# valeoai/PAFUSE

Measured on AMD Instinct MI355X. Metric: hypotheses/sec through DDIM loop (H3WB 133-kp, P=20, T=10), higher is better.
Workload: dtype bf16x3 (every fp32 GEMM operand as the exact sum of three bf16 slices, six bf16 MFMA products per fp32-equivalent product, fp32 accumulate; activations, LayerNorm, softmax, attention and everything in memory fp32; the residual stream stored centred on its row means)

## Files before the change

### pafuse_amd/csrc/kernels.hpp

```cpp
#pragma once
#include <hip/hip_runtime.h>
#include <stdint.h>

#include <utility>

namespace pafuse {

typedef float f32x16 __attribute__((ext_vector_type(16)));
typedef float f32x4 __attribute__((ext_vector_type(4)));

constexpr int BK = 32;
constexpr int LDK = 36;

typedef __bf16 bf16x8 __attribute__((ext_vector_type(8)));
__device__ __forceinline__ bf16x8 to_bf16x8(const f32x4 lo, const f32x4 hi) {
    bf16x8 v;
#pragma unroll
    for (int i = 0; i < 4; ++i) v[i] = (__bf16)lo[i], v[4 + i] = (__bf16)hi[i];
    return v;
}

#ifdef PAFUSE_MFMA_K8
typedef __bf16 bf16x4_t __attribute__((ext_vector_type(4)));
typedef short s16x4_t __attribute__((ext_vector_type(4)));
// ... 1238 lines not shown
            }
            static_for<NG>([&](auto G) {
                constexpr int g = decltype(G)::value;
                constexpr int nt = g % NT;
                constexpr bool SPL = g < NT && ABL < 3 && NS2 == 2;
                constexpr int q0 = SPL ? (4 * nt) / NT : 0, q1 = SPL ? (4 * (nt + 1)) / NT : 0;
                if constexpr (g + 1 < NG) {
                    load_w(std::integral_constant<int, g + 1>{});
                    if constexpr (g == 0 && NS2 == 2) {
                        asm volatile("s_waitcnt lgkmcnt(3)"
                                     : "+v"(wf[0][0]), "+v"(wf[0][1]), "+v"(wf[0][2]), "+v"(b_lo), "+v"(b_hi));
    #pragma unroll
                        for (int q = 0; q < 4; ++q) {
                            sp[q].x0 = __builtin_bit_cast(float, q < 2 ? b_lo[2 * q] : b_hi[2 * q - 4]);
                            sp[q].x1 = __builtin_bit_cast(float, q < 2 ? b_lo[2 * q + 1] : b_hi[2 * q - 3]);
                        }
                    } else {
                        asm volatile("s_waitcnt lgkmcnt(3)" : "+v"(wf[g & 1][0]), "+v"(wf[g & 1][1]), "+v"(wf[g & 1][2]));
                    }
                } else {
                    asm volatile("s_waitcnt lgkmcnt(0)" : "+v"(wf[g & 1][0]), "+v"(wf[g & 1][1]), "+v"(wf[g & 1][2]));
                }
                const u32x4(&w)[3] = wf[g & 1];
                auto mm = [&](int wi, int ai) {
                    PAFUSE_PIN_ACC(acc[nt]);
                    acc[nt] = mfma_bf16_k16(__builtin_bit_cast(bf16x8, w[wi]), __builtin_bit_cast(bf16x8, cur[ai]), acc[nt]);
                };
                auto pins = [&]() {
    #pragma unroll
                    for (int q = q0; q < q1; ++q) PAFUSE_PIN_PAIR(sp[q]);
                };
                pins();
                mm(0, 2);
                {
                    constexpr int PER = (CNT + NG - 1) / NG, j0 = g * PER, j1 = (g + 1) * PER < CNT ? (g + 1) * PER : CNT;
                    if constexpr (j0 < j1 && ABL < 2) {
                        asm volatile("" ::: "memory");
                        if (refill) {
    #pragma unroll
                            for (int j = j0; j < j1; ++j) issue_piece(kn, stn, j);
                        }
                        asm volatile("" ::: "memory");
                    }
                }
    #pragma unroll
                for (int q = q0; q < q1; ++q) sp[q].template stage<0>();
                pins();
                mm(2, 0);
    #pragma unroll
                for (int q = q0; q < q1; ++q) sp[q].template stage<1>();
                pins();
                mm(1, 1);
    #pragma unroll
                for (int q = q0; q < q1; ++q) sp[q].template stage<2>();
                pins();
                mm(0, 1);
    #pragma unroll
                for (int q = q0; q < q1; ++q) sp[q].template stage<3>();
                pins();
                mm(1, 0);
    #pragma unroll
                for (int q = q0; q < q1; ++q) {
                    sp[q].template stage<4>();
                    nxt[0][q] = sp[q].s0, nxt[1][q] = sp[q].s1, nxt[2][q] = sp[q].s2;
                }
                pins();
                mm(0, 0);
                if constexpr (g == NT - 1 && ABL < 3 && NS2 == 2) cur[0] = nxt[0], cur[1] = nxt[1], cur[2] = nxt[2];
                if constexpr (g == NT - 1 && ABL >= 3 && NS2 == 2) {
    #pragma unroll
                    for (int q = 0; q < 4; ++q)
                        cur[0][q] = cur[2][q] = __builtin_bit_cast(uint32_t, sp[q].x0), cur[1][q] = __builtin_bit_cast(uint32_t, sp[q].x1);
                }
            });
    #undef PAFUSE_PIN_ACC
    #undef PAFUSE_PIN_PAIR
            __builtin_amdgcn_s_setprio(0);
        }
    }
    PAFUSE_STAMP(1);
    __syncthreads();
    constexpr int VEC = EPI == EPI_BIAS ? 0 : (7 * BM * WN + 3) / 4 * 4;
    if constexpr (VEC > 0) {
        static_assert((size_t)(VEC + 5 * BN) * sizeof(float) <= (size_t)NSTAGE * T::STAGE_BYTES, "epilogue vectors must fit the ring");
        const float* const src[5] = {p.bias, p.post_w, p.post_b, p.next_w, p.next_b};
#pragma unroll
        for (int v = 0; v < 5; ++v)
            if (src[v])
                for (int i = tid; i < BN / 4; i += T::NTHR)
                    *reinterpret_cast<f32x4*>(smem + VEC + v * BN + 4 * i) = *reinterpret_cast<const f32x4*>(src[v] + n0 + 4 * i);
        __syncthreads();
    }
    if constexpr (ABL == 4) {
        float sacc = 0.f;
#pragma unroll
        for (int nt = 0; nt < NT; ++nt)
#pragma unroll
            for (int i = 0; i < 16; ++i) sacc += acc[nt][i];
        if (sacc == 123.456f) p.out[0] = sacc;
        return;
    }
    if constexpr (EPI == EPI_ROWLN && SLAB) {
        constexpr size_t RINGF = (size_t)NSTAGE * T::STAGE_BYTES / sizeof(float);
        constexpr auto need = [](int nth) { return (size_t)VEC + 5 * BN + (size_t)NW * 32 * (32 * nth + 4); };
        constexpr int NTH = (NT % 2 == 0 && need(2) <= RINGF) ? 2 : 1;
        static_assert(need(NTH) <= RINGF, "epilogue scratch must fit the ring");
        epilogue_rows_h<WN, NT, BM, NW, NTH, false, 2>(acc, p, m0, n0, wm, wn, r, h, wave, lane, smem, 1.0f);
    } else {
        epilogue_row_per_lane<WN, NT, BM, EPI, VEC>(acc, p, m0, n0, wm, wn, r, h, smem);
    }
}

template <int WM, int WN, int NT, int EPI, int NSTAGE, int MINW, int ABL = 0, int BKC = 32>
__global__ void __launch_bounds__(WM* WN * 64, MINW) gemm_dma_kernel(const GemmParams p) {
    PAFUSE_XQ_GUARD();
    extern __shared__ __attribute__((aligned(16))) float smem[];
    gemm_dma_tile<WM, WN, NT, EPI, NSTAGE, ABL, BKC>(p, blockIdx.x, gridDim.x, smem);
}

constexpr int GROUP_MAX = 4;
struct GroupedGemmParams {
    GemmParams p[GROUP_MAX];
    int first[GROUP_MAX + 1];
    int n;
};

template <int EPI>
__global__ void __launch_bounds__(256, 2) grouped_rowln_kernel(const GroupedGemmParams g) {
    PAFUSE_XQ_GUARD();
    extern __shared__ __attribute__((aligned(16))) float smem[];
    const int b = blockIdx.x;
    int s = 0;
#pragma unroll
    for (int i = 1; i < GROUP_MAX; ++i)
        if (i < g.n && b >= g.first[i]) s = i;
    const GemmParams& p = g.p[s];
    const int lb = b - g.first[s], nb = g.first[s + 1] - g.first[s];
    switch (p.N) {
        case 384: gemm_dma_tile<2, 2, 6, EPI, 2, 0, 16, false>(p, lb, nb, smem); break;
        case 256: gemm_dma_tile<2, 2, 4, EPI, 2, 0, 16, false>(p, lb, nb, smem); break;
        case 224: gemm_dma_tile<4, 1, 7, EPI, 2, 0, 16, false>(p, lb, nb, smem); break;
        default: break;
    }
}

struct AttnParams {
    const float* qkv;
    float* o;
    uint8_t* o_h;
    int64_t nseq;
    int L, C, heads, d;
    int64_t group, group_stride, seq_stride, tok_stride;
    float scale;
};

template <int ITEMS>
__device__ __forceinline__ void attn_item(int64_t i, int64_t nseq, int heads, int64_t& seq, int& head) {
    if (nseq % 8 == 0 && ((nseq / 8) * heads) % ITEMS == 0) {
        const int64_t blk = i / ITEMS;
        const int lo = (int)(blk % 8);
        const int64_t u = (blk / 8) * ITEMS + (i % ITEMS);
        head = (int)(u % heads);
        seq = (u / heads) * 8 + lo;
    } else {
        seq = i / heads;
        head = (int)(i % heads);
    }
}

template <int LP, int DP, int NW>
__global__ void __launch_bounds__(NW * 64) attn_kernel(const AttnParams p) {
    PAFUSE_XQ_GUARD();
    constexpr int QT = LP / 16, KT = LP / 16, CT = DP / 16, SD = DP / 16, ITEMS = NW / QT, LDV = DP + 4;
    constexpr int NTHR = NW * 64, C4 = DP / 4;
    static_assert(NW % QT == 0, "waves must be a multiple of the query tiles");
    extern __shared__ __attribute__((aligned(16))) float smem[];
    float* Ks = smem;
    float* Vs = smem + ITEMS * LP * LDV;
    const int tid = threadIdx.x, lane = tid & 63, wave = tid >> 6;
    const int64_t nitems = p.nseq * p.heads;
    const int C3 = 3 * p.C;

    const int il = wave / QT, qt = wave % QT;
    const int64_t item = (int64_t)blockIdx.x * ITEMS + il;
    const bool mine = item < nitems;
    int64_t seq = 0;
    int head = 0;
    if (mine) attn_item<ITEMS>(item, p.nseq, p.heads, seq, head);
    const int64_t base = (seq / p.group) * p.group_stride + (seq % p.group) * p.seq_stride;
    const int l15 = lane & 15, g = lane >> 4;
    f32x4 qf[SD];
    {
        const int q = qt * 16 + l15;
#pragma unroll
        for (int s = 0; s < SD; ++s) {
            qf[s] = f32x4{0.f, 0.f, 0.f, 0.f};
            if (mine && q < p.L && 16 * s + 4 * g < p.d)
                qf[s] = *reinterpret_cast<const f32x4*>(p.qkv + (base + q * p.tok_stride) * C3 + head * p.d + 16 * s +
                                                        4 * g);
        }
    }
    for (int sl = 0; sl < ITEMS; ++sl) {
        const int64_t it2 = (int64_t)blockIdx.x * ITEMS + sl;
        const bool ok = it2 < nitems;
        int64_t seq2 = 0;
        int head2 = 0;
        if (ok) attn_item<ITEMS>(it2, p.nseq, p.heads, seq2, head2);
        const int64_t base2 = (seq2 / p.group) * p.group_stride + (seq2 % p.group) * p.seq_stride;
        for (int idx = tid; idx < LP * C4; idx += NTHR) {
            const int t = idx / C4, c4 = idx % C4;
            f32x4 kv = {0.f, 0.f, 0.f, 0.f}, vv = {0.f, 0.f, 0.f, 0.f};
            if (ok && t < p.L && c4 * 4 < p.d) {
                const float* src = p.qkv + (base2 + t * p.tok_stride) * C3 + head2 * p.d + c4 * 4;
                kv = *reinterpret_cast<const f32x4*>(src + p.C);
                vv = *reinterpret_cast<const f32x4*>(src + 2 * p.C);
            }
            *reinterpret_cast<f32x4*>(Ks + (sl * LP + t) * LDV + c4 * 4) = kv;
            *reinterpret_cast<f32x4*>(Vs + (sl * LP + t) * LDV + c4 * 4) = vv;
        }
    }
    __syncthreads();
    if (!mine) return;
    const float* Kb = Ks + il * LP * LDV;
    const float* Vb = Vs + il * LP * LDV;
    f32x4 sc[KT];
#pragma unroll
    for (int kt = 0; kt < KT; ++kt) sc[kt] = f32x4{0.f, 0.f, 0.f, 0.f};
#pragma unroll
    for (int s = 0; s < SD; ++s) {
        f32x4 kf[KT];
#pragma unroll
        for (int kt = 0; kt < KT; ++kt)
            kf[kt] = *reinterpret_cast<const f32x4*>(Kb + (kt * 16 + l15) * LDV + 16 * s + 4 * g);
#pragma unroll
        for (int j = 0; j < 4; ++j)
#pragma unroll
            for (int kt = 0; kt < KT; ++kt)
                sc[kt] = __builtin_amdgcn_mfma_f32_16x16x4f32(kf[kt][j], qf[s][j], sc[kt], 0, 0, 0);
    }
    float mx = -INFINITY;
#pragma unroll
    for (int kt = 0; kt < KT; ++kt)
#pragma unroll
        for (int reg = 0; reg < 4; ++reg) {
            const int key = kt * 16 + 4 * g + reg;
            const float v = key < p.L ? sc[kt][reg] * p.scale : -INFINITY;
            sc[kt][reg] = v;
            mx = fmaxf(mx, v);
        }
    mx = fmaxf(mx, __shfl_xor(mx, 16));
    mx = fmaxf(mx, __shfl_xor(mx, 32));
    float sum = 0.f;
#pragma unroll
    for (int kt = 0; kt < KT; ++kt)
#pragma unroll
        for (int reg = 0; reg < 4; ++reg) {
            const float e = __builtin_amdgcn_exp2f((sc[kt][reg] - mx) * 1.44269504088896340736f);
            sc[kt][reg] = e;
            sum += e;
        }
    sum += __shfl_xor(sum, 16);
    sum += __shfl_xor(sum, 32);
    const float inv = 1.0f / sum;
#pragma unroll
    for (int kt = 0; kt < KT; ++kt)
#pragma unroll
        for (int reg = 0; reg < 4; ++reg) sc[kt][reg] *= inv;

    f32x4 oc[CT];
#pragma unroll
    for (int ct = 0; ct < CT; ++ct) oc[ct] = f32x4{0.f, 0.f, 0.f, 0.f};
#pragma unroll
    for (int kt = 0; kt < KT; ++kt)
#pragma unroll
        for (int reg = 0; reg < 4; ++reg) {
            const float* vrow = Vb + (kt * 16 + 4 * g + reg) * LDV + l15;
#pragma unroll
            for (int ct = 0; ct < CT; ++ct)
                oc[ct] = __builtin_amdgcn_mfma_f32_16x16x4f32(vrow[ct * 16], sc[kt][reg], oc[ct], 0, 0, 0);
        }
    const int q = qt * 16 + l15;
    if (q < p.L) {
        if (p.o_h) {
            uint8_t* const hrow = p.o_h + (base + q * p.tok_stride) * p.C * 4;
#pragma unroll
            for (int ct = 0; ct < CT; ++ct)
                if (ct * 16 + 4 * g < p.d) {
                    const int c = head * p.d + ct * 16 + 4 * g;
                    hsplit_store4(hrow + (c >> 3) * 32, c & 4, oc[ct]);
                }
            return;
        }
        float* orow = p.o + (base + q * p.tok_stride) * p.C + head * p.d + 4 * g;
#pragma unroll
        for (int ct = 0; ct < CT; ++ct)
            if (ct * 16 + 4 * g < p.d) *reinterpret_cast<f32x4*>(orow + ct * 16) = oc[ct];
    }
}

constexpr int ATTN_LONG_LP = 256;
template <int DP>
__global__ void __launch_bounds__(1024) attn_long_kernel(const AttnParams p) {
    PAFUSE_XQ_GUARD();
    constexpr int LP = ATTN_LONG_LP, T = LP / 16, SD = DP / 16, CT = DP / 16, LDV = DP + 4, C4 = DP / 4;
    extern __shared__ __attribute__((aligned(16))) float smem[];
    float* Ks = smem;
    float* Vs = smem + LP * LDV;
    const int tid = threadIdx.x, lane = tid & 63, w = tid >> 6, l15 = lane & 15, g = lane >> 4;
    int64_t seq;
    int head;
    attn_item<1>((int64_t)blockIdx.x, p.nseq, p.heads, seq, head);
    const int64_t base = (seq / p.group) * p.group_stride + (seq % p.group) * p.seq_stride;
    const int C3 = 3 * p.C, nt = (p.L + 15) / 16;
    f32x4 qf[SD];
    {
        const int q = 16 * w + l15;
#pragma unroll
        for (int s = 0; s < SD; ++s) {
            qf[s] = f32x4{0.f, 0.f, 0.f, 0.f};
            if (q < p.L && 16 * s + 4 * g < p.d)
                qf[s] = *reinterpret_cast<const f32x4*>(p.qkv + (base + (int64_t)q * p.tok_stride) * C3 + head * p.d + 16 * s + 4 * g);
        }
    }
    for (int idx = tid; idx < nt * 16 * C4; idx += 1024) {
        const int t = idx / C4, c4 = idx % C4;
        f32x4 kv = {0.f, 0.f, 0.f, 0.f}, vv = {0.f, 0.f, 0.f, 0.f};
        if (t < p.L && c4 * 4 < p.d) {
            const float* src = p.qkv + (base + (int64_t)t * p.tok_stride) * C3 + head * p.d + c4 * 4;
            kv = *reinterpret_cast<const f32x4*>(src + p.C);
            vv = *reinterpret_cast<const f32x4*>(src + 2 * p.C);
        }
        *reinterpret_cast<f32x4*>(Ks + t * LDV + c4 * 4) = kv;
        *reinterpret_cast<f32x4*>(Vs + t * LDV + c4 * 4) = vv;
    }
    __syncthreads();
    if (w >= nt) return;
    f32x4 sc[T];
#pragma unroll
    for (int kt = 0; kt < T; ++kt) {
        sc[kt] = f32x4{0.f, 0.f, 0.f, 0.f};
        if (kt < nt) {
#pragma unroll
            for (int s = 0; s < SD; ++s) {
                const f32x4 kf = *reinterpret_cast<const f32x4*>(Ks + (kt * 16 + l15) * LDV + 16 * s + 4 * g);
#pragma unroll
                for (int j = 0; j < 4; ++j) sc[kt] = __builtin_amdgcn_mfma_f32_16x16x4f32(kf[j], qf[s][j], sc[kt], 0, 0, 0);
            }
        }
    }
    float mx = -INFINITY;
#pragma unroll
    for (int kt = 0; kt < T; ++kt)
#pragma unroll
        for (int reg = 0; reg < 4; ++reg) {
            const float v = kt * 16 + 4 * g + reg < p.L ? sc[kt][reg] * p.scale : -INFINITY;
            sc[kt][reg] = v;
            mx = fmaxf(mx, v);
        }
    mx = fmaxf(mx, __shfl_xor(mx, 16));
    mx = fmaxf(mx, __shfl_xor(mx, 32));
    float sum = 0.f;
#pragma unroll
    for (int kt = 0; kt < T; ++kt)
#pragma unroll
        for (int reg = 0; reg < 4; ++reg) {
            const float e = __builtin_amdgcn_exp2f((sc[kt][reg] - mx) * 1.44269504088896340736f);
            sc[kt][reg] = e;
            sum += e;
        }
    sum += __shfl_xor(sum, 16);
    sum += __shfl_xor(sum, 32);
    const float inv = 1.0f / sum;
    f32x4 oc[CT];
#pragma unroll
    for (int ct = 0; ct < CT; ++ct) oc[ct] = f32x4{0.f, 0.f, 0.f, 0.f};
#pragma unroll
    for (int kt = 0; kt < T; ++kt)
        if (kt < nt) {
#pragma unroll
            for (int reg = 0; reg < 4; ++reg) {
                const float pr = sc[kt][reg] * inv;
                const float* vrow = Vs + (kt * 16 + 4 * g + reg) * LDV + l15;
#pragma unroll
                for (int ct = 0; ct < CT; ++ct) oc[ct] = __builtin_amdgcn_mfma_f32_16x16x4f32(vrow[ct * 16], pr, oc[ct], 0, 0, 0);
            }
        }
    const int q = 16 * w + l15;
    if (q < p.L) {
        float* orow = p.o + (base + (int64_t)q * p.tok_stride) * p.C + head * p.d + 4 * g;
#pragma unroll
        for (int ct = 0; ct < CT; ++ct)
            if (ct * 16 + 4 * g < p.d) *reinterpret_cast<f32x4*>(orow + ct * 16) = oc[ct];
    }
}

struct FqaParams {
    GemmParams g;
    float* o;
    int64_t nseq;
    int L, C, heads, d, nseq_tile;
    int64_t group, group_stride, seq_stride, tok_stride;
    float scale;
};

template <int LP, int DP>
struct FqaTile {
    static constexpr int NB = 3 * DP / 16, LDV = DP + 4, ROWS = 128 + (LP == 48 ? 4 : 0);
    static constexpr int STAGE_BYTES = Tile16<NB>::STAGE_BYTES, QKV_BYTES = 3 * ROWS * LDV * 4;
    static constexpr int LDS_BYTES = STAGE_BYTES > QKV_BYTES ? STAGE_BYTES : QKV_BYTES;
};

template <int LP, int DP>
__global__ void __launch_bounds__(256, 2) fqa_kernel(const FqaParams fp) {
    PAFUSE_XQ_GUARD();
    using FT = FqaTile<LP, DP>;
    constexpr int NB = FT::NB, LDV = FT::LDV, ROWS = FT::ROWS;
    using T = Tile16<NB>;
    constexpr int A_LD = T::A_LD, W_LD = T::W_LD, NTHR = T::NTHR;
    extern __shared__ __attribute__((aligned(16))) float smem[];
    const GemmParams& p = fp.g;
    uint8_t* const As = reinterpret_cast<uint8_t*>(smem);
    uint8_t* const Ws = As + T::A_BYTES;
    const int tid = threadIdx.x, lane = tid & 63, wave = tid >> 6;
    const int c = lane & 15, qd = lane >> 4;
    const int L = fp.L, NSEQ = fp.nseq_tile;
    const int64_t ntiles = (fp.nseq + NSEQ - 1) / NSEQ;
    const int xcd = blockIdx.x & 7, idx = blockIdx.x >> 3;
    const int64_t tile = (int64_t)(idx / fp.heads) * 8 + xcd;
    const int head = idx % fp.heads;
    if (tile >= ntiles) return;
    const int K = p.K, nk = K / 32;
    const int64_t seq0 = tile * NSEQ;
    const int64_t last_seq = fp.nseq - 1;
    auto token_of = [&](int r) -> int64_t {
        int sl = r / L, t = r - sl * L;
        if (sl >= NSEQ) sl = NSEQ - 1, t = L - 1;
        int64_t sq = seq0 + sl;
        if (sq > last_seq) sq = last_seq;
        return (sq / fp.group) * fp.group_stride + (sq % fp.group) * fp.seq_stride + t * fp.tok_stride;
    };

    const float* a_ptr[A_LD];
    int a_dst[A_LD];
#pragma unroll
    for (int i = 0; i < A_LD; ++i) {
        const int g = 2 * wave + (i >> 1), j = 4 * (i & 1) + qd;
        a_ptr[i] = p.A + token_of(16 * g + c) * K + 4 * j;
        a_dst[i] = g * 2048 + (j & 1) * 1024 + ((j >> 1) * 16 + c) * 16;
    }
// ... 2602 lines not shown
```

### pafuse_amd/csrc/pafuse_hip.hip

```cpp
#include "../../include/pafuse_hip.h"

#include <hip/hip_runtime.h>

#include <algorithm>
#include <cmath>
#include <cstdarg>
#include <cstdio>
#include <cstdlib>
#include <cstring>
#include <type_traits>

#include "kernels.hpp"
#include "hgemm.hpp"
#include "xgemm.hpp"
#include "sgemm.hpp"
#include "train_kernels.hpp"

using namespace pafuse;

namespace {

thread_local char g_err[512] = "";

int fail(int code, const char* fmt, ...) {
// ... 372 lines not shown
        if (p.N % 64 == 0) return launch_gemm<4, 1, 2, EPI_BIAS, 1, 4, 0, 2>(p, s);
    }
    if (p.M <= 0) return PAFUSE_OK;
    if (p.K % BK || p.N % 32 || p.K <= 0 || p.N <= 0)
        return fail(PAFUSE_E_SHAPE, "linear: N=%d K=%d must be positive multiples of 32", p.N, p.K);
    if ((p.out_act || p.dact_u) && ((p.N % 64 && !(p.mode == MODE_BF16X3 && p.wlayout == WLAYOUT_M16)) || mode_images(p.mode) || p.ln_in || p.act))
        return fail(PAFUSE_E_ARG, "linear: out_act / dact_u need N %% 64 == 0 and a plain fp32 or bf16x3 product");
    if (p.mode == MODE_F16X2) return hgemm_bias(p, s);
    if (p.mode == MODE_BF16X3_IMAGES) return xgemm_bias(p, s);
#ifdef PAFUSE_QKV_32X32
    p.wlayout = WLAYOUT_PLAIN;
#endif
#ifndef PAFUSE_NO_STRIP
    if (strip2_ok(p)) return strip2_bias(p, s);
#endif
    if (p.mode == MODE_BF16X3 && p.wlayout == WLAYOUT_M16) {
        if (p.N % 128 == 0) return launch_gemm16<8, 3>(p, s);
        if (p.N % 96 == 0) return launch_gemm16<6, 3>(p, s);
        if (p.N % 112 == 0) return launch_gemm16<7, 3>(p, s);
        if (p.N % 64 == 0) return launch_gemm16<4, 4>(p, s);
        return launch_gemm16<2, 4>(p, s);
    }
    if (p.mode == MODE_BF16X3) {
        if (p.N % 128 == 0 && p.M >= 4096) return launch_gemm<4, 1, 4, EPI_BIAS, 1, PAFUSE_FC1_MINW, 0, 2>(p, s);
        if (p.N % 64 == 0) return launch_gemm<4, 1, 2, EPI_BIAS, 1, 4, 0, 2>(p, s);
        if (p.N % 96 == 0) return launch_gemm<4, 1, 3, EPI_BIAS, 1, 1, 1, 2>(p, s);
        return launch_gemm<4, 1, 1, EPI_BIAS, 1, 1, 0, 2>(p, s);
    }
    if (p.mode != MODE_F32) {
        if (p.N % 64 == 0) return launch_gemm<4, 1, 2, EPI_BIAS, 1, 5, 0, 1>(p, s);
        if (p.N % 96 == 0) return launch_gemm<4, 1, 3, EPI_BIAS, 1, 1, 1, 1>(p, s);
        return launch_gemm<4, 1, 1, EPI_BIAS, 1, 1, 0, 1>(p, s);
    }
    if (p.N % 64 == 0) return launch_gemm<4, 1, 2, EPI_BIAS, 1, 5>(p, s);
    if (p.N % 96 == 0) return launch_gemm<4, 1, 3, EPI_BIAS, 1, 1, 1>(p, s);
    return launch_gemm<4, 1, 1, EPI_BIAS, 1>(p, s);
}

template <int EPI>
int gemm_rowln_as(const GemmParams& p0, hipStream_t s) {
    GemmParams p = p0;
    if (p.mode == MODE_BF16X3 && (debug_f32_mask() & 2)) p.mode = MODE_F32;
    if (p.M <= 0) return PAFUSE_OK;
    if (p.K % BK || p.K <= 0) return fail(PAFUSE_E_SHAPE, "rowln: K=%d must be a positive multiple of 32", p.K);
    if (p.mode == MODE_F16X2 || p.mode == MODE_BF16X3_IMAGES) {
        if constexpr (EPI == EPI_ROWLN) return p.mode == MODE_F16X2 ? hgemm_rowln(p, s) : xgemm_rowln(p, s);
        else return fail(PAFUSE_E_ARG, "training has no image-pipeline kernels");
    }
    if constexpr (EPI == EPI_ROWLN_TRAIN) {
        if (p.mode == MODE_BF16X3) {
            switch (p.N) {
                case 384: return launch_gemm_dma<2, 2, 6, EPI, 2, 2, 16>(p, s);
                case 256: return launch_gemm_dma<2, 2, 4, EPI, 2, 2, 16>(p, s);
                case 224: if (p.M >= 4096) return launch_gemm_dma<4, 1, 7, EPI, 2, 2, 16>(p, s); break;
                default: break;
            }
            p.mode = MODE_F32;
        }
    }
    if constexpr (EPI == EPI_ROWLN) {
        if (p.mode == MODE_BF16X3) {
            switch (p.N) {
                case 384: return launch_gemm_dma<2, 2, 6, EPI, 2, 2, 16>(p, s);
                case 256: return launch_gemm_dma<2, 2, 4, EPI, 2, 2, 16>(p, s);
                case 288: return launch_gemm_dma<2, 3, 3, EPI, 2, 2, 16>(p, s);
                case 224:
                    return p.M >= 4096 ? launch_gemm_dma<4, 1, 7, EPI, 2, 2, 16>(p, s) : launch_gemm_dma<2, 1, 7, EPI, 2, 2, 16>(p, s);
                case 128: return launch_gemm<1, 4, 1, EPI, 1, 1, 1, 2>(p, s);
                case 64: return launch_gemm<1, 2, 1, EPI, 1, 1, 1, 2>(p, s);
                default: break;
            }
        } else if (p.mode != MODE_F32) {
            switch (p.N) {
                case 384: return launch_gemm<1, 4, 3, EPI, 1, 1, 1, 1>(p, s);
                case 288: return launch_gemm<1, 3, 3, EPI, 1, 1, 1, 1>(p, s);
                case 256: return launch_gemm<2, 2, 4, EPI, 1, 2, 1, 1>(p, s);
                case 224: return launch_gemm<1, 7, 1, EPI, 1, 1, 1, 1>(p, s);
                case 128: return launch_gemm<1, 4, 1, EPI, 1, 1, 1, 1>(p, s);
                case 64: return launch_gemm<1, 2, 1, EPI, 1, 1, 1, 1>(p, s);
                default: break;
            }
        }
    }
    switch (p.N) {
        case 384: return launch_gemm<1, 4, 3, EPI, 1, 1, 1>(p, s);
        case 288: return launch_gemm<1, 3, 3, EPI, 1, 1, 1>(p, s);
        case 256: return launch_gemm<2, 2, 4, EPI, 1, 2, 1>(p, s);
        case 224: return launch_gemm<1, 7, 1, EPI, 1, 1, 1>(p, s);
        case 128: return launch_gemm<1, 4, 1, EPI, 1, 1, 1>(p, s);
        case 64: return launch_gemm<1, 2, 1, EPI, 1, 1, 1>(p, s);
        default: return fail(PAFUSE_E_SHAPE, "no whole-row kernel for channel width %d (have 64,128,224,256,288,384)", p.N);
    }
}

int gemm_rowln(const GemmParams& p, hipStream_t s) { return gemm_rowln_as<EPI_ROWLN>(p, s); }
int gemm_rowln_train(const GemmParams& p, hipStream_t s) { return gemm_rowln_as<EPI_ROWLN_TRAIN>(p, s); }

bool group_ok_rowln(const GemmParams& p) {
    return p.mode == MODE_BF16X3 && p.Wsplit && (p.N == 384 || p.N == 256 || (p.N == 224 && p.M >= 4096)) && p.K % 16 == 0 && p.K > 0 &&
           !(debug_f32_mask() & 2);
}

template <bool ROWLN>
int gemm_group(const GemmParams* ps, int n, hipStream_t s, bool shared_grids) {
    bool ok = ROWLN && shared_grids && n >= 2 && n <= GROUP_MAX;
    for (int i = 0; i < n && ok; ++i) ok = ps[i].M > 0 && group_ok_rowln(ps[i]);
    if (!ok) {
        for (int i = 0; i < n; ++i) {
            const int rc = ROWLN ? gemm_rowln(ps[i], s) : gemm_bias(ps[i], s);
            if (rc) return rc;
        }
        return PAFUSE_OK;
    }
    int order[GROUP_MAX];
    double cost[GROUP_MAX];
    int64_t tiles[GROUP_MAX];
    for (int i = 0; i < n; ++i) {
        const GemmParams& p = ps[i];
        int bm, bn;
        bm = p.N == 224 ? 128 : 64, bn = p.N;
        tiles[i] = (p.M + bm - 1) / bm * (p.N / bn);
        cost[i] = (double)bm * bn * p.K;
        order[i] = i;
    }
    std::sort(order, order + n, [&](int a, int b) { return cost[a] > cost[b]; });
    GroupedGemmParams g{};
    g.n = n;
    int64_t first = 0;
    for (int k = 0; k < n; ++k) {
        g.p[k] = ps[order[k]];
        g.first[k] = (int)first;
        first += (tiles[order[k]] + 7) / 8 * 8;
        if (first > 0x7fffffff) return fail(PAFUSE_E_ARG, "grouped gemm grid out of range");
    }
    g.first[n] = (int)first;
    for (int k = n + 1; k <= GROUP_MAX; ++k) g.first[k] = (int)first;
    constexpr size_t lds = 2 * DmaTile<2, 2, 6, 16>::STAGE_BYTES;
    static_assert(lds >= 2 * DmaTile<2, 2, 4, 16>::STAGE_BYTES && lds >= 2 * DmaTile<4, 1, 7, 16>::STAGE_BYTES && lds <= 80 * 1024, "LDS");
    return launch<grouped_rowln_kernel<EPI_ROWLN>>("grouped_rowln_kernel", (unsigned)first, 256, lds, s, g);
}

bool width_supported(int C) { return C == 384 || C == 288 || C == 256 || C == 224 || C == 128 || C == 64; }

template <int LP, int DP, int NW>
int launch_attn(const AttnParams& p, hipStream_t s) {
    constexpr int ITEMS = NW / (LP / 16);
    constexpr size_t lds = (size_t)2 * ITEMS * LP * (DP + 4) * sizeof(float);
    const int64_t nitems = p.nseq * p.heads;
    const int64_t grid = (nitems + ITEMS - 1) / ITEMS;
    if (grid > 0x7fffffff) return fail(PAFUSE_E_ARG, "attention grid out of range");
    return launch<attn_kernel<LP, DP, NW>>("attn_kernel", (unsigned)grid, NW * 64, lds, s, p);
}

template <int DP>
int launch_attn_long(const AttnParams& p, hipStream_t s) {
    constexpr size_t lds = (size_t)2 * ATTN_LONG_LP * (DP + 4) * sizeof(float);
    static_assert(lds <= 160 * 1024, "LDS");
    const int64_t grid = p.nseq * p.heads;
    if (grid > 0x7fffffff) return fail(PAFUSE_E_ARG, "attention grid out of range");
    return launch<attn_long_kernel<DP>>("attn_long_kernel", (unsigned)grid, 1024, lds, s, p);
}

int attention(const AttnParams& p, hipStream_t s) {
    if (p.nseq <= 0) return PAFUSE_OK;
#ifdef PAFUSE_ABL_NO_ATTENTION
    return PAFUSE_OK;
#endif
    if (p.d % 4 || p.d > 48 || p.L > ATTN_LONG_LP || p.L <= 0)
        return fail(PAFUSE_E_SHAPE, "attention: head dim %d (need %%4, <=48) / length %d (need <=%d)", p.d, p.L, ATTN_LONG_LP);
    if (p.L > 144) {
        if (p.o_h) return fail(PAFUSE_E_SHAPE, "attention: no f16x2 image output for sequences of %d > 144 tokens: use mode 2", p.L);
        return p.d <= 32 ? launch_attn_long<32>(p, s) : launch_attn_long<48>(p, s);
    }
    const int dp = p.d <= 32 ? 32 : 48;
    const int lp = p.L <= 32 ? 32 : (p.L <= 48 ? 48 : (p.L <= 80 ? 80 : 144));
    if (lp == 144)
        return dp == 32 ? launch_attn<144, 32, 9>(p, s) : launch_attn<144, 48, 9>(p, s);
    if (dp == 32) {
        if (lp == 32) return launch_attn<32, 32, 4>(p, s);
        if (lp == 48) return launch_attn<48, 32, 6>(p, s);
        return launch_attn<80, 32, 5>(p, s);
    }
    if (lp == 32) return launch_attn<32, 48, 4>(p, s);
    if (lp == 48) return launch_attn<48, 48, 6>(p, s);
    return launch_attn<80, 48, 5>(p, s);
}

constexpr size_t RANGE_FLAG_BYTES = 256;

struct PartBuffers {
    float *x, *xn, *o, *wide;
    int eb;
    float* temb;
    float* pred;
    float* stats;
};

size_t part_buffer_bytes(int64_t M, int C, int B, int eb = 4) {
    return align_up((size_t)M * C * 4) + 2 * align_up((size_t)M * C * eb) + align_up((size_t)M * 3 * C * 4) + align_up((size_t)B * C * 4) +
           align_up((size_t)M * 3 * 4) + align_up((size_t)M * 2 * 4);
}

char* carve_part(char* base, int64_t M, int C, int B, PartBuffers& pb, int eb = 4) {
    pb.eb = eb;
    pb.x = (float*)base;
    base += align_up((size_t)M * C * 4);
    pb.xn = (float*)base;
    base += align_up((size_t)M * C * eb);
    pb.o = (float*)base;
    base += align_up((size_t)M * C * eb);
    pb.wide = (float*)base;
    base += align_up((size_t)M * 3 * C * 4);
    pb.temb = (float*)base;
    base += align_up((size_t)B * C * 4);
    pb.pred = (float*)base;
    base += align_up((size_t)M * 3 * 4);
    pb.stats = (float*)base;
    base += align_up((size_t)M * 2 * 4);
    return base;
}

PartBuffers offset_rows(const PartBuffers& pb, int64_t row0, int C) {
    PartBuffers o = pb;
    const int64_t img = row0 * C * pb.eb / 4;
    o.x = pb.x + row0 * C, o.xn = pb.xn + img, o.o = pb.o + img, o.wide = pb.wide + row0 * 3 * C;
    o.pred = pb.pred + row0 * 3;
    o.stats = pb.stats + row0 * 2;
    return o;
}

static bool ln_folded(const pafuse_mixste2_weights* w) { return w->ste[0].qkv_lt != nullptr; }
static bool h_residual_only(const pafuse_mixste2_weights* w) { return mode_images(w->operand_bf16) && ln_folded(w) && !w->keep_f32_residual; }

static void embed_outputs(EmbedParams& e, int mode, bool folded, bool h_only, float* x, float* xn, void* image, float* stats,
                          int64_t row0, int64_t nrows) {
    e.x = h_only ? nullptr : x, e.xn = xn;
    e.stats = folded ? stats : nullptr;
    e.xh = mode_images(mode) ? reinterpret_cast<uint8_t*>(image) : nullptr;
    e.x_image = mode == MODE_BF16X3_IMAGES;
    e.centre_x = mode == MODE_BF16X3 && folded;
    e.row0 = row0, e.nrows = nrows;
}

int check_weights(const pafuse_mixste2_weights* w, bool training = false) {
    if (!w) return fail(PAFUSE_E_ARG, "null weights");
    static_assert(EMBED_NV * 128 >= 384, "embed kernel covers the widest part");
    if (w->in_chans != 5) return fail(PAFUSE_E_SHAPE, "in_chans must be 5, got %d", w->in_chans);
    if (w->depth < 1 || w->depth > PAFUSE_MAX_DEPTH) return fail(PAFUSE_E_SHAPE, "depth %d out of range", w->depth);
    if (!width_supported(w->channels)) return fail(PAFUSE_E_SHAPE, "channel width %d has no kernel", w->channels);
    if (w->heads <= 0 || w->channels % w->heads) return fail(PAFUSE_E_SHAPE, "heads %d !| C %d", w->heads, w->channels);
    const int d = w->channels / w->heads;
    if (d % 4 || d > 48) return fail(PAFUSE_E_SHAPE, "head dim %d unsupported", d);
    if (w->joints < 1 || w->joints > 144 || w->frames < 1 || w->frames > ATTN_LONG_LP)
        return fail(PAFUSE_E_SHAPE, "sequence lengths J=%d F=%d: J must be in 1..144, F in 1..%d", w->joints, w->frames, ATTN_LONG_LP);
    if (w->operand_bf16 == MODE_F16X2 && w->frames > 144)
        return fail(PAFUSE_E_SHAPE, "f16x2: no attention form for clips of %d > 144 frames: use mode 2", w->frames);
    if (!mode_valid(w->operand_bf16)) return fail(PAFUSE_E_ARG, "matrix-product mode %d", w->operand_bf16);
    if (mode_images(w->operand_bf16)) {
        const int hidden = w->mlp_hidden > 0 ? w->mlp_hidden : 2 * w->channels;
        if (!hgemm_width(w->channels) || !hgemm_plain_n(3 * w->channels) || !hgemm_plain_n(hidden) || hidden % 32)
            return fail(PAFUSE_E_SHAPE, "the image pipelines (f16x2, bf16x3 on images) serve the widths 224 / 256 / 384 with an MLP hidden "
                                        "width that is a multiple of 128 or 224 (got C = %d, hidden = %d): use mode 2", w->channels, hidden);
    }
    if (w->operand_bf16 == MODE_BF16X3_IMAGES && !training) {
        for (int i = 0; i < w->depth; ++i)
            for (const pafuse_block_weights* b : {&w->ste[i], &w->tte[i]})
                if (!b->qkv_hs || !b->qkv_hb) return fail(PAFUSE_E_ARG, "bf16x3 on images needs the head-major qkv image of every block (qkv_hs, qkv_hb)");
        if (!xfqa_has(w->joints, d, w->heads) || !xfqa_has(w->frames, d, w->heads))
            return fail(PAFUSE_E_SHAPE, "bf16x3 on images: no fused qkv + attention form for sequences of %d / %d tokens at head dim %d, %d heads: "
                                        "use mode 2", w->joints, w->frames, d, w->heads);
    }
    if (w->mlp_hidden < 0 || (w->mlp_hidden > 0 && (w->mlp_hidden % 32 || w->mlp_hidden > 3 * w->channels)))
        return fail(PAFUSE_E_SHAPE, "mlp hidden width %d must be a multiple of 32 and at most 3C = %d", w->mlp_hidden, 3 * w->channels);
    if (!(w->qk_scale >= 0.f)) return fail(PAFUSE_E_ARG, "qk_scale must be positive (0 = head_dim^-0.5)");
    if (training && (w->operand_bf16 == MODE_BF16 || mode_images(w->operand_bf16)))
        return fail(PAFUSE_E_ARG, "training runs fp32 ('f32') or split-precision ('bf16x3') products");
    if (mode_split(w->operand_bf16) && !training)
        for (int i = 0; i < w->depth; ++i)
            for (const pafuse_block_weights* b : {&w->ste[i], &w->tte[i]})
                if ((!b->qkv_ws && w->operand_bf16 != MODE_BF16X3_IMAGES) || !b->proj_ws || !b->fc1_ws || !b->fc2_ws)
                    return fail(PAFUSE_E_ARG, "split-precision mode needs the pre-split image of every linear weight "
                                              "(pafuse_split_weights)");
    const bool fold = ln_folded(w);
    for (int i = 0; i < w->depth; ++i)
        for (const pafuse_block_weights* b : {&w->ste[i], &w->tte[i]}) {
            const int set = (b->qkv_lt != nullptr) + (b->fc1_lt != nullptr);
            if (set != (fold ? 2 : 0)) return fail(PAFUSE_E_ARG, "folded-LayerNorm vectors (qkv_lt, fc1_lt) must be set in every block or in none");
        }
    if (fold && !mode_split(w->operand_bf16)) return fail(PAFUSE_E_ARG, "the folded LayerNorm exists in the split-precision modes only");
    return PAFUSE_OK;
}

struct BlockTail {
    const float *post_w, *post_b;
    float post_eps;
    const float* pos;
    int posJ, posF;
    const float *next_w, *next_b;
    float next_eps;
    const float *head_w, *head_b;
    float* out_head;
};

struct BlockLaunch {
    GemmParams qkv, proj, fc1, fc2;
    AttnParams attn;
    FqaParams fqa;
    bool fused;
    MlpParams mlp;
    bool mlp_fused;
};

BlockLaunch make_block(const pafuse_block_weights& bw, const PartBuffers& pb, int64_t M, int C, int heads, int64_t nseq, int L,
                       int64_t group, int64_t group_stride, int64_t seq_stride, int64_t tok_stride, const BlockTail& tail,
                       int mode, int hidden = 0, float qk_scale = 0.f, bool fold = false, bool keep_f32_residual = false) {
    if (hidden <= 0) hidden = 2 * C;
    BlockLaunch b{};
    float* const stats = pb.stats;
    const bool hp = mode_images(mode);
    uint8_t* const xn_h = reinterpret_cast<uint8_t*>(pb.xn);
    const bool h_residual = hp && fold && !keep_f32_residual;
    GemmParams& g = b.qkv;
    g.A = pb.xn, g.W = bw.qkv_w, g.bias = bw.qkv_b, g.out = pb.wide, g.M = M, g.N = 3 * C, g.K = C, g.act = 0;
    g.mode = mode, g.Wsplit = (const uint8_t*)bw.qkv_ws, g.wlayout = WLAYOUT_M16;
    if (fold) g.A = pb.x, g.ln_in = stats, g.bias = bw.qkv_lt;
    if (hp) g.Ah = xn_h, g.Wh = (const uint8_t*)bw.qkv_ws;
// ... 1932 lines not shown
```

Measured before the change: 102.8.

## Add run-based attention kernel with register prefetch and shape-specialised templates

Adds attn_run_kernel, which handles RUN item groups per workgroup. The next group's Q/K/V is loaded into registers while the current one is computed, then stashed into a double-buffered LDS region. It also specialises on common sequence lengths and head dims (27/28, 42, 68, 24/48) to skip padded MFMA tiles, preloads V into registers before softmax, and uses 3 waves instead of 6 for L≤48. With ATTN_RUN=1 the prefetch path is inactive, so the gain rests on the specialisation and reduced padding; the extra register arrays may raise pressure. Timing-stamp instrumentation is added under a compile flag.

```diff
diff --git a/pafuse_amd/csrc/kernels.hpp b/pafuse_amd/csrc/kernels.hpp
--- a/pafuse_amd/csrc/kernels.hpp
+++ b/pafuse_amd/csrc/kernels.hpp
@@ -1414,7 +1414,14 @@
     int L, C, heads, d;
     int64_t group, group_stride, seq_stride, tok_stride;
     float scale;
-};
+#ifdef PAFUSE_STAMPS
+    unsigned long long* stamps;
+#endif
+};
+
+__host__ __device__ inline bool attn_xcd_order(int64_t nseq, int heads, int items) {
+    return nseq % 8 == 0 && ((nseq / 8) * heads) % items == 0;
+}
 
 template <int ITEMS>
 __device__ __forceinline__ void attn_item(int64_t i, int64_t nseq, int heads, int64_t& seq, int& head) {
@@ -1433,6 +1440,10 @@
 template <int LP, int DP, int NW>
 __global__ void __launch_bounds__(NW * 64) attn_kernel(const AttnParams p) {
     PAFUSE_XQ_GUARD();
+#ifdef PAFUSE_STAMPS
+    if (p.stamps && (threadIdx.x & 63) == 0 && PAFUSE_STAMP_SLOTS >= 7)
+        p.stamps[((size_t)blockIdx.x * NW + (threadIdx.x >> 6)) * PAFUSE_STAMP_SLOTS + 6] = pafuse_stamp();
+#endif
     constexpr int QT = LP / 16, KT = LP / 16, CT = DP / 16, SD = DP / 16, ITEMS = NW / QT, LDV = DP + 4;
     constexpr int NTHR = NW * 64, C4 = DP / 4;
     static_assert(NW % QT == 0, "waves must be a multiple of the query tiles");
@@ -1462,6 +1473,11 @@
                                                         4 * g);
         }
     }
+    PAFUSE_STAMP(0);
+#ifdef PAFUSE_STAMPS
+    if (p.stamps && lane == 0 && PAFUSE_STAMP_SLOTS >= 6)
+        p.stamps[((size_t)blockIdx.x * NW + wave) * PAFUSE_STAMP_SLOTS + 5] = __builtin_amdgcn_s_memrealtime();
+#endif
     for (int sl = 0; sl < ITEMS; ++sl) {
         const int64_t it2 = (int64_t)blockIdx.x * ITEMS + sl;
         const bool ok = it2 < nitems;
@@ -1482,6 +1498,7 @@
         }
     }
     __syncthreads();
+    PAFUSE_STAMP(1);
     if (!mine) return;
     const float* Kb = Ks + il * LP * LDV;
     const float* Vb = Vs + il * LP * LDV;
@@ -1541,6 +1558,10 @@
             for (int ct = 0; ct < CT; ++ct)
                 oc[ct] = __builtin_amdgcn_mfma_f32_16x16x4f32(vrow[ct * 16], sc[kt][reg], oc[ct], 0, 0, 0);
         }
+#ifdef PAFUSE_STAMPS
+    asm volatile("" ::"v"(oc[0]), "v"(oc[CT - 1]));
+#endif
+    PAFUSE_STAMP(2);
     const int q = qt * 16 + l15;
     if (q < p.L) {
         if (p.o_h) {
@@ -1557,6 +1578,188 @@
 #pragma unroll
         for (int ct = 0; ct < CT; ++ct)
             if (ct * 16 + 4 * g < p.d) *reinterpret_cast<f32x4*>(orow + ct * 16) = oc[ct];
+    }
+#ifdef PAFUSE_STAMPS
+    asm volatile("s_waitcnt vmcnt(0)" ::: "memory");
+    PAFUSE_STAMP(3);
+    if (p.stamps && lane == 0 && PAFUSE_STAMP_SLOTS >= 5)
+        p.stamps[((size_t)blockIdx.x * NW + wave) * PAFUSE_STAMP_SLOTS + 4] = __builtin_amdgcn_s_memrealtime();
+#endif
+}
+
+template <int LP, int DP, int NW, int RUN, int LC = 0, int DC = 0>
+__global__ void __launch_bounds__(NW * 64) attn_run_kernel(const AttnParams p) {
+    PAFUSE_XQ_GUARD();
+    constexpr int QT = LP / 16, KT = LP / 16, CT = DP / 16, SD = DP / 16, ITEMS = NW / QT, LDV = DP + 4;
+    constexpr int NTHR = NW * 64, C4 = DP / 4, NLD = (LP * C4 + NTHR - 1) / NTHR, BUF = 2 * ITEMS * LP * LDV;
+    static_assert(NW % QT == 0, "waves must be a multiple of the query tiles");
+    extern __shared__ __attribute__((aligned(16))) float smem[];
+    const int tid = threadIdx.x, lane = tid & 63, wave = tid >> 6;
+    const int il = wave / QT, qt = wave % QT, l15 = lane & 15, g = lane >> 4;
+    const int64_t nitems = p.nseq * p.heads, ngroups = (nitems + ITEMS - 1) / ITEMS;
+    const int C3 = 3 * p.C;
+    constexpr int LS = LC ? LC : LP, DSK = DC ? DC : DP, NT = (LS + 15) / 16;
+    const int L = LC ? LC : p.L, d = DC ? DC : p.d;
+    const bool xcd_order = attn_xcd_order(p.nseq, p.heads, ITEMS);
+    const int64_t wg = blockIdx.x;
+    auto group_of = [&](int r) { return xcd_order ? ((wg >> 3) * RUN + r) * 8 + (wg & 7) : wg * RUN + r; };
+
+    int64_t base_n = 0;
+    int head_n = 0;
+    bool mine_n = false;
+    f32x4 qn[SD], kr[ITEMS][NLD], vr[ITEMS][NLD];
+    auto issue = [&](int64_t grp) {
+        int64_t base2[ITEMS];
+        int head2[ITEMS];
+        bool ok2[ITEMS];
+#pragma unroll
+        for (int sl = 0; sl < ITEMS; ++sl) {
+            const int64_t it2 = grp * ITEMS + sl;
+            int64_t seq2 = 0;
+            head2[sl] = 0;
+            ok2[sl] = it2 < nitems;
+            if (ok2[sl]) attn_item<ITEMS>(it2, p.nseq, p.heads, seq2, head2[sl]);
+            base2[sl] = (seq2 / p.group) * p.group_stride + (seq2 % p.group) * p.seq_stride;
+            if (sl == il) base_n = base2[sl], head_n = head2[sl], mine_n = ok2[sl];
+        }
+        const int q = qt * 16 + l15;
+#pragma unroll
+        for (int s = 0; s < SD; ++s) {
+            qn[s] = f32x4{0.f, 0.f, 0.f, 0.f};
+            if (mine_n && q < L && 16 * s + 4 * g < d)
+                qn[s] = *reinterpret_cast<const f32x4*>(p.qkv + (base_n + q * p.tok_stride) * C3 + head_n * d + 16 * s + 4 * g);
+        }
+#pragma unroll
+        for (int sl = 0; sl < ITEMS; ++sl)
+#pragma unroll
+            for (int i = 0; i < NLD; ++i) {
+                const int idx = tid + i * NTHR, t = idx / C4, c4 = idx % C4;
+                kr[sl][i] = f32x4{0.f, 0.f, 0.f, 0.f};
+                vr[sl][i] = f32x4{0.f, 0.f, 0.f, 0.f};
+                if (ok2[sl] && t < L && c4 * 4 < d) {
+                    const float* src = p.qkv + (base2[sl] + t * p.tok_stride) * C3 + head2[sl] * d + c4 * 4;
+                    kr[sl][i] = *reinterpret_cast<const f32x4*>(src + p.C);
+                    vr[sl][i] = *reinterpret_cast<const f32x4*>(src + 2 * p.C);
+                }
+            }
+    };
+    auto stash = [&](float* buf) {
+#pragma unroll
+        for (int sl = 0; sl < ITEMS; ++sl)
+#pragma unroll
+            for (int i = 0; i < NLD; ++i) {
+                const int idx = tid + i * NTHR, t = idx / C4, c4 = idx % C4;
+                if (t < 16 * NT) {
+                    *reinterpret_cast<f32x4*>(buf + (sl * LP + t) * LDV + c4 * 4) = kr[sl][i];
+                    *reinterpret_cast<f32x4*>(buf + ((ITEMS + sl) * LP + t) * LDV + c4 * 4) = vr[sl][i];
+                }
+            }
+    };
+
+    if (group_of(0) >= ngroups) return;
+    issue(group_of(0));
+    stash(smem);
+#pragma unroll
+    for (int r = 0; r < RUN; ++r) {
+        if (group_of(r) < ngroups) {
+            __syncthreads();
+            const int64_t base = base_n;
+            const int head = head_n;
+            const bool mine = mine_n;
+            f32x4 qf[SD];
+#pragma unroll
+            for (int s = 0; s < SD; ++s) qf[s] = qn[s];
+            const bool more = r + 1 < RUN && group_of(r + 1) < ngroups;
+            if (more) issue(group_of(r + 1));
+            if (mine && qt < NT) {
+                const float* Kb = smem + (r & 1) * BUF + il * LP * LDV;
+                const float* Vb = Kb + ITEMS * LP * LDV;
+                f32x4 sc[KT];
+#pragma unroll
+                for (int kt = 0; kt < KT; ++kt) sc[kt] = f32x4{0.f, 0.f, 0.f, 0.f};
+#pragma unroll
+                for (int s = 0; s < SD; ++s) {
+                    if (16 * s >= DSK) break;
+                    f32x4 kf[KT];
+#pragma unroll
+                    for (int kt = 0; kt < KT; ++kt) {
+                        kf[kt] = f32x4{0.f, 0.f, 0.f, 0.f};
+                        if (kt < NT) kf[kt] = *reinterpret_cast<const f32x4*>(Kb + (kt * 16 + l15) * LDV + 16 * s + 4 * g);
+                    }
+#pragma unroll
+                    for (int j = 0; j < 4; ++j)
+                        if (16 * s + j < DSK) {
+#pragma unroll
+                            for (int kt = 0; kt < KT; ++kt)
+                                if (kt < NT) sc[kt] = __builtin_amdgcn_mfma_f32_16x16x4f32(kf[kt][j], qf[s][j], sc[kt], 0, 0, 0);
+                        }
+                }
+                float vv[KT][4][CT];
+#pragma unroll
+                for (int kt = 0; kt < KT; ++kt)
+#pragma unroll
+                    for (int reg = 0; reg < 4; ++reg)
+#pragma unroll
+                        for (int ct = 0; ct < CT; ++ct) {
+                            vv[kt][reg][ct] = 0.f;
+                            if (kt < NT) vv[kt][reg][ct] = Vb[(kt * 16 + 4 * g + reg) * LDV + l15 + ct * 16];
+                        }
+                __builtin_amdgcn_sched_barrier(0);
+                float mx = -INFINITY;
+#pragma unroll
+                for (int kt = 0; kt < KT; ++kt)
+#pragma unroll
+                    for (int reg = 0; reg < 4; ++reg) {
+                        const int key = kt * 16 + 4 * g + reg;
+                        float sv = sc[kt][reg] * p.scale;
+                        asm("" : "+v"(sv));
+                        const float v = key < L ? sv : -INFINITY;
+                        sc[kt][reg] = v;
+                        mx = fmaxf(mx, v);
+                    }
+                mx = fmaxf(mx, __shfl_xor(mx, 16));
+                mx = fmaxf(mx, __shfl_xor(mx, 32));
+                float sum = 0.f;
+#pragma unroll
+                for (int kt = 0; kt < KT; ++kt)
+#pragma unroll
+                    for (int reg = 0; reg < 4; ++reg) {
+                        const float e = __builtin_amdgcn_exp2f((sc[kt][reg] - mx) * 1.44269504088896340736f);
+                        sc[kt][reg] = e;
+                        sum += e;
+                    }
+                sum += __shfl_xor(sum, 16);
+                sum += __shfl_xor(sum, 32);
+                const float inv = 1.0f / sum;
+#pragma unroll
+                for (int kt = 0; kt < KT; ++kt)
+#pragma unroll
+                    for (int reg = 0; reg < 4; ++reg) sc[kt][reg] *= inv;
+
+                f32x4 oc[CT];
+#pragma unroll
+                for (int ct = 0; ct < CT; ++ct) oc[ct] = f32x4{0.f, 0.f, 0.f, 0.f};
+#pragma unroll
+                for (int kt = 0; kt < KT; ++kt) {
+                    if (kt >= NT) break;
+#pragma unroll
+                    for (int reg = 0; reg < 4; ++reg)
+                        if (16 * kt + reg < LS) {
+#pragma unroll
+                            for (int ct = 0; ct < CT; ++ct)
+                                oc[ct] = __builtin_amdgcn_mfma_f32_16x16x4f32(vv[kt][reg][ct], sc[kt][reg], oc[ct], 0, 0, 0);
+                        }
+                }
+                const int q = qt * 16 + l15;
+                if (q < L) {
+                    float* orow = p.o + (base + q * p.tok_stride) * p.C + head * d + 4 * g;
+#pragma unroll
+                    for (int ct = 0; ct < CT; ++ct)
+                        if (ct * 16 + 4 * g < d) *reinterpret_cast<f32x4*>(orow + ct * 16) = oc[ct];
+                }
+            }
+            if (more) stash(smem + ((r + 1) & 1) * BUF);
+        }
     }
 }
 
diff --git a/pafuse_amd/csrc/pafuse_hip.hip b/pafuse_amd/csrc/pafuse_hip.hip
--- a/pafuse_amd/csrc/pafuse_hip.hip
+++ b/pafuse_amd/csrc/pafuse_hip.hip
@@ -548,6 +548,43 @@
     return launch<attn_kernel<LP, DP, NW>>("attn_kernel", (unsigned)grid, NW * 64, lds, s, p);
 }
 
+template <int LP, int DP, int NW, int RUN, int LC = 0, int DC = 0>
+int launch_attn_run(const AttnParams& p, hipStream_t s) {
+    constexpr int ITEMS = NW / (LP / 16);
+    constexpr size_t lds = (size_t)(RUN > 1 ? 2 : 1) * 2 * ITEMS * LP * (DP + 4) * sizeof(float);
+    static_assert(lds <= 80 * 1024, "LDS");
+    const int64_t nitems = p.nseq * p.heads;
+    const int64_t ngroups = (nitems + ITEMS - 1) / ITEMS;
+    const int64_t grid = attn_xcd_order(p.nseq, p.heads, ITEMS) ? (ngroups / 8 + RUN - 1) / RUN * 8 : (ngroups + RUN - 1) / RUN;
+    if (grid > 0x7fffffff) return fail(PAFUSE_E_ARG, "attention grid out of range");
+    return launch<attn_run_kernel<LP, DP, NW, RUN, LC, DC>>("attn_run_kernel", (unsigned)grid, NW * 64, lds, s, p);
+}
+
+constexpr int ATTN_RUN = 1;
+int attention_runs(const AttnParams& p, hipStream_t s) {
+    constexpr int R = ATTN_RUN;
+    if (p.d <= 32) {
+        if (p.L <= 32) {
+            if (p.L == 27 && p.d == 28) return launch_attn_run<32, 32, 4, R, 27, 28>(p, s);
+            if (p.L == 27 && p.d == 32) return launch_attn_run<32, 32, 4, R, 27, 32>(p, s);
+            return launch_attn_run<32, 32, 4, R>(p, s);
+        }
+        if (p.L <= 48) {
+            if (p.L == 42 && p.d == 32) return launch_attn_run<48, 32, 3, R, 42, 32>(p, s);
+            return launch_attn_run<48, 32, 3, R>(p, s);
+        }
+        if (p.L == 68 && p.d == 28) return launch_attn_run<80, 32, 5, R, 68, 28>(p, s);
+        return launch_attn_run<80, 32, 5, R>(p, s);
+    }
+    if (p.L <= 32) {
+        if (p.L == 24 && p.d == 48) return launch_attn_run<32, 48, 4, R, 24, 48>(p, s);
+        if (p.L == 27 && p.d == 48) return launch_attn_run<32, 48, 4, R, 27, 48>(p, s);
+        return launch_attn_run<32, 48, 4, R>(p, s);
+    }
+    if (p.L <= 48) return launch_attn_run<48, 48, 3, R>(p, s);
+    return launch_attn_run<80, 48, 5, R>(p, s);
+}
+
 template <int DP>
 int launch_attn_long(const AttnParams& p, hipStream_t s) {
     constexpr size_t lds = (size_t)2 * ATTN_LONG_LP * (DP + 4) * sizeof(float);
@@ -568,6 +605,9 @@
         if (p.o_h) return fail(PAFUSE_E_SHAPE, "attention: no f16x2 image output for sequences of %d > 144 tokens: use mode 2", p.L);
         return p.d <= 32 ? launch_attn_long<32>(p, s) : launch_attn_long<48>(p, s);
     }
+#ifndef PAFUSE_ATTN_NO_RUNS
+    if (!p.o_h && p.L <= 80) return attention_runs(p, s);
+#endif
     const int dp = p.d <= 32 ? 32 : 48;
     const int lp = p.L <= 32 ? 32 : (p.L <= 48 ? 48 : (p.L <= 80 ? 80 : 144));
     if (lp == 144)
```

Result: no change. 103.5, median of 6 (+0.7%).
